# jameshensman/pyvb

Hardware: AMD Instinct MI355X
Metric: VB update iterations/sec (T=10k, D=64, N=1024 LDS); ELBO rel-err vs NumPy (higher is better)
Workload: dtype f64; 1 GPU; LDS T=10000 D=64 K=64, 1024 replicates per GPU (BASELINE configs[2]); replicates_total=1024, parallelism=replicates sharded over 1 GPU(s), collective=none (1 GPU), degraded=False

## Files before the change

### pyvb_amd/csrc/api.hip

```cpp
#include "common.h"
#include <cstdarg>
#include <cstdio>
#include <cstdlib>
#include <cstring>
#include <cmath>
#include <vector>
#include <mutex>
#include <dlfcn.h>

static thread_local char g_err[512] = "";

void pyvb_set_error(const char* fmt, ...) {
    va_list ap; va_start(ap, fmt);
    vsnprintf(g_err, sizeof(g_err), fmt, ap);
    va_end(ap);
}

int pyvb_hip_fail(hipError_t e, const char* what, const char* file, int line) {
    pyvb_set_error("HIP error %d (%s) in %s at %s:%d", (int)e, hipGetErrorString(e), what, file, line);
    return PYVB_E_HIP;
}

TimedLaunch::TimedLaunch(pyvb_lds* h_, int k_, hipStream_t s_) : h(h_), slot(-1), s(s_ ? s_ : h_->stream) {
    if (!h->timing) return;
// ... 610 lines not shown
        const double* Sm = S.data() + m * D * D;
        double s = 0.0;
        for (size_t j = 0; j < D && s == s; ++j) {
            for (size_t i = j; i < D; ++i) {
                double v = Sm[i * D + j];
                for (size_t k = 0; k < j; ++k) v -= L[i * D + k] * L[j * D + k];
                if (i == j) {
                    if (!(v > 0.0)) { s = NAN; break; }
                    L[j * D + j] = sqrt(v);
                    s += log(v);
                } else L[i * D + j] = v / L[j * D + j];
            }
        }
        lnd[m] = s;
    }
    HIPCHK(hipMemcpyAsync(h->lnd_x, lnd.data(), lnd.size() * sizeof(double), hipMemcpyHostToDevice, h->stream));
    HIPCHK(hipStreamSynchronize(h->stream));
    h->st.lnd_x_pending = false;
    return PYVB_OK;
}

static int ensure_gains(pyvb_lds* h) {
    if (h->st.gains_valid) return PYVB_OK;
    int rc;
    if (h->dense) {
        if ((rc = ensure_expect(h))) return rc;
        if ((rc = launch_dense_pre(h))) return rc;
    }
    if ((rc = launch_prep(h))) return rc;
    h->st.gains_formed();
    return PYVB_OK;
}

static void adopt_classes(pyvb_lds* h) {
    double* t = h->Sigma; h->Sigma = h->Sigma_new; h->Sigma_new = t;
    t = h->qld_x; h->qld_x = h->qld_x_new; h->qld_x_new = t;
    t = h->lnd_x; h->lnd_x = h->lnd_x_new; h->lnd_x_new = t;
    h->st.classes_adopted(h->n_active < h->N);
}

static int ensure_stats(pyvb_lds* h) {
    LdsState& st = h->st;
    if (st.stats_valid) return PYVB_OK;
    if (!st.classes_valid) {
        pyvb_set_error("the posterior covariances of the X_t are undefined before the first complete sweep "
                       "(run pyvb_lds_sweep, or give them with pyvb_lds_set_posterior_classes)");
        return PYVB_E_STALE;
    }
    if (st.mixed_cov || (st.gains_valid && st.fresh_count != 0 && st.fresh_count != h->T)) {
        pyvb_set_error("%d of %d X_t were updated since the parameters changed: their covariances differ; sweep all states first",
                       st.fresh_count, h->T);
        return PYVB_E_STALE;
    }
    int rc = launch_stats(h, !st.sxx_valid);
    if (rc) return rc;
    if ((rc = launch_moments(h, st.sxx_valid))) return rc;
    st.stats_valid = true;
    return PYVB_OK;
}

static int ensure_resid(pyvb_lds* h, int which) {
    bool& valid = which == 0 ? h->st.resQ_valid : h->st.resR_valid;
    if (valid) return PYVB_OK;
    int rc = ensure_stats(h);
    if (rc) return rc;
    if ((rc = h->dense ? launch_wresid(h, which, 0, h->st.sg_valid[which]) : launch_resid(h, which))) return rc;
    valid = true;
    return PYVB_OK;
}

static int sweep(pyvb_lds* h, int direction, bool keep_x) {
    int rc = ensure_gains(h);
    if (rc) return rc;
    const bool read_cache = direction == PYVB_BACKWARD && h->st.u_valid;
    if ((rc = launch_sweep(h, direction, h->st.cur, read_cache, keep_x))) return rc;
    h->st.sweep_ran(direction, read_cache, !h->big);
    if (h->st.all_fresh()) adopt_classes(h);
    return PYVB_OK;
}

int pyvb_lds_sweep(pyvb_lds* h, int direction) {
    ENTER(h);
    ARGCHK(direction == PYVB_FORWARD || direction == PYVB_BACKWARD, "direction must be PYVB_FORWARD or PYVB_BACKWARD");
    IDLE(h);
    return sweep(h, direction, true);
}

int pyvb_lds_update_x(pyvb_lds* h, int t) {
    ENTER(h);
    ARGCHK(t >= 0 && t < h->T, "t out of range");
    IDLE(h);
    int rc = ensure_gains(h);
    if (rc) return rc;
    if ((rc = launch_step(h, t))) return rc;
    h->st.x_changed();
    if (h->st.node_fresh(t)) adopt_classes(h);
    return PYVB_OK;
}

int pyvb_lds_update_columns(pyvb_lds* h, int which, int col_begin, int col_end) {
    ENTER(h);
    ARGCHK(which == 0 || which == 1, "which must be 0 (A) or 1 (C)");
    ARGCHK(col_begin >= 0 && col_begin < col_end && col_end <= h->D, "bad column range");
    IDLE(h);
    int rc = ensure_stats(h);
    if (rc) return rc;
    if (h->dense) {
        if ((rc = ensure_expect(h))) return rc;
        if ((rc = launch_cols_dense(h, which, col_begin, col_end))) return rc;
    } else if ((rc = launch_cols(h, which, col_begin, col_end))) return rc;
    h->st.columns_updated(which, h->dense && col_begin == 0 && col_end == h->D);
    return PYVB_OK;
}

int pyvb_lds_update_A(pyvb_lds* h) { ARGCHK(h, "handle is NULL"); return pyvb_lds_update_columns(h, 0, 0, h->D); }
int pyvb_lds_update_C(pyvb_lds* h) { ARGCHK(h, "handle is NULL"); return pyvb_lds_update_columns(h, 1, 0, h->D); }

static int update_noise(pyvb_lds* h, int which) {
    int rc;
    if (h->dense) {
        if ((rc = ensure_stats(h))) return rc;
        if ((rc = launch_wresid(h, which, 1, h->st.sg_valid[which]))) return rc;
    } else {
        if ((rc = ensure_resid(h, which))) return rc;
        if ((rc = launch_noise(h, which))) return rc;
    }
    h->st.noise_updated(which);
    return PYVB_OK;
}
// ... 310 lines not shown
```

### pyvb_amd/csrc/common.h

```cpp
#pragma once
#include <cstdint>
#include "host.h"

struct pyvb_comm;
typedef double d4 __attribute__((ext_vector_type(4)));
typedef double d2 __attribute__((ext_vector_type(2)));

struct Layout {
    int D, K, DT, KT, DP, KP, DS, KS;
    int QR;
    size_t oFn, oBn, oGp;
    size_t oS0, oS2, oqr, ow0;
    size_t gains_total;
    size_t stats_total;
    size_t oSxx, oSx1x, oSyx;
};

__host__ __device__ static inline int xpos(int d) { return (d & ~15) | ((d & 3) << 2) | ((d >> 2) & 3); }

__host__ __device__ static inline size_t pos_nat(int i, int j, int S) {
    return ((size_t)((i >> 4) * S + (j >> 2)) * 64) + (j & 3) * 16 + (i & 15);
}
__host__ __device__ static inline size_t pos_perm(int i, int j, int S) {
    int s = 2 * (j >> 3) + (j & 1), q = (j & 7) >> 1;
// ... 50 lines not shown
    double *A_mean, *A_var, *C_mean, *C_var;
    double *Q_a, *Q_b, *R_a, *R_b;
    double *qld_A, *qld_C;
    double *lnd_A, *lnd_C;
    int bound;
    Priors pri;
    double *pri_block;
    double *Sigma, *qld_x;
    double *Sigma_new, *qld_x_new;
    double *lnd_x, *lnd_x_new;
    double *gains;
    double *scratch;
    int *warm;
    double *zeros;
    double *trash;
    double *U;
    double *stats; int nchunk, chunk_len;
    int W;
    double *sxx;
    double *mom;
    double *resQ, *resR;
    double *elbo, *elbo_sum;
    int *status;
    unsigned char *active;
    unsigned char *active_host;
    int n_active;
    int *status_host, *reported;
    LdsState st;
    DeviceBuffers mem;
    bool timing; KernelTimer timers[PYVB_K_COUNT]; int timing_errors;
    pyvb_comm* comm; int rank, world;
    bool dense;
    double *Q_w, *R_w;
    double *Qbar, *Rbar;
    double *lnd;
    double *QA, *RC;
    double *trA, *trC;
    double *A_cov, *C_cov;
    double *SyyF;
    double *RQ, *RR;
    double *ldm;
    double *SG;
    bool has_missing;
    double *Yobs, *Yvar, *Yqld, *Yent;
    double *Ylnd, *YentX;
    double *Yld, *YcovS;
    hipStream_t side;
    hipEvent_t ev_params, ev_elbo;
    bool elbo_in_flight;
    double* elbo_hist; int hist_count;
};
#define PYVB_ELBO_HISTORY 4096

int launch_prep(pyvb_lds* h);
int launch_sweep(pyvb_lds* h, int direction, int src, bool read_cache, bool keep_x);
int launch_step(pyvb_lds* h, int t);
int launch_syy(pyvb_lds* h);
int launch_permute(pyvb_lds* h, const double* src, double* dst, int to_internal);
int launch_carry(pyvb_lds* h, const double* src, double* dst, size_t per);
int launch_stats(pyvb_lds* h, bool with_sxx);
int launch_moments(pyvb_lds* h, bool sxx_from_sweep);
int launch_observe(pyvb_lds* h);
int launch_cols(pyvb_lds* h, int which, int c0, int c1, int fuse = 0);
int launch_resid(pyvb_lds* h, int which);
int launch_noise(pyvb_lds* h, int which);
int launch_elbo(pyvb_lds* h, hipStream_t stream = nullptr);
int launch_elbo_sum(pyvb_lds* h, double* out = nullptr, hipStream_t stream = nullptr);
int launch_prep_big(pyvb_lds* h);
int big_prepare_kernels();
int launch_sweep_big(pyvb_lds* h, int direction, int src, bool cached);
int launch_step_big(pyvb_lds* h, int t);
int launch_stats_big(pyvb_lds* h);
int launch_cols_big(pyvb_lds* h, int which, int c0, int c1, int fuse);
int launch_wexpect(pyvb_lds* h);
int launch_dense_pre(pyvb_lds* h);
int launch_cols_dense(pyvb_lds* h, int which, int c0, int c1);
int launch_wresid(pyvb_lds* h, int which, int update, bool use_sg);
int launch_syy_full(pyvb_lds* h);
int launch_elbo_dense(pyvb_lds* h, hipStream_t stream = nullptr);
int launch_colvar_to_cov(pyvb_lds* h);
int launch_cov_to_colvar(pyvb_lds* h);
int launch_cov_observe(pyvb_lds* h);
int launch_cov_convert(pyvb_lds* h, int which, double* dense, int n0, int count, int to_packed);
int launch_wexpect_big(pyvb_lds* h);
int launch_dense_pre_big(pyvb_lds* h);
int launch_cols_dense_big(pyvb_lds* h, int which, int c0, int c1);
int launch_wresid_big(pyvb_lds* h, int which, int update, bool use_sg);
int launch_syy_full_big(pyvb_lds* h);
int launch_missing_init(pyvb_lds* h, const double* Yq0, const double* Yrowvar0);
int launch_impute(pyvb_lds* h);
int launch_syy_missing(pyvb_lds* h);
int launch_impute_dense(pyvb_lds* h);
int launch_missing_ent_dense(pyvb_lds* h, int diag_cov);

struct pyvb_comm {
    void* nccl;
    pyvb_host_allreduce_fn fn; void* user;
    double* host; size_t cap;
};
int pyvb_comm_create(pyvb_comm** comm, const char id[128], int rank, int world);
int pyvb_comm_create_host(pyvb_comm** comm, pyvb_host_allreduce_fn fn, void* user);
void pyvb_comm_free(pyvb_comm* comm);
int pyvb_allreduce_f64(pyvb_comm* comm, double* buf, size_t count, hipStream_t stream);

#define PYVB_EVENT_POOL 2048
struct EventPair { hipEvent_t e0, e1; int kernel; };
struct TimedLaunch {
    pyvb_lds* h; int slot; hipStream_t s;
    TimedLaunch(pyvb_lds* h_, int k_, hipStream_t s_ = nullptr);
    ~TimedLaunch();
};
void pyvb_timing_resolve(pyvb_lds* h);
```

### pyvb_amd/csrc/host.h

```cpp
#pragma once
#include <hip/hip_runtime.h>
#include <cstddef>
#include <cstring>
#include <vector>
#include "../../include/pyvb_hip.h"

void pyvb_set_error(const char* fmt, ...);
int pyvb_hip_fail(hipError_t e, const char* what, const char* file, int line);
#define HIPCHK(x) do { hipError_t _e = (x); if (_e != hipSuccess) return pyvb_hip_fail(_e, #x, __FILE__, __LINE__); } while (0)
#define ARGCHK(cond, msg) do { if (!(cond)) { pyvb_set_error("%s", msg); return PYVB_E_ARG; } } while (0)
#define ENTER_DEVICE(h) do { ARGCHK(h, "handle is NULL"); HIPCHK(hipSetDevice((h)->device)); } while (0)
#define CREATE_TRY(x, DESTROY, h) do { rc = (x); if (rc != PYVB_OK) { DESTROY(h); return rc; } } while (0)
#define CREATE_TRYHIP(x, DESTROY, h) do { hipError_t _e = (x); if (_e != hipSuccess) { rc = pyvb_hip_fail(_e, #x, __FILE__, __LINE__); DESTROY(h); return rc; } } while (0)

struct DeviceBuffers {
    std::vector<void*> owned;
    int alloc(void** p, size_t bytes, int fill_byte = 0) {
        HIPCHK(hipMalloc(p, bytes));
        owned.push_back(*p);
        HIPCHK(hipMemset(*p, fill_byte, bytes));
        return PYVB_OK;
    }
    int zeros(double** p, size_t n) { return alloc((void**)p, n * sizeof(double)); }
    void release(void* p) {
        for (size_t i = 0; i < owned.size(); ++i)
            if (owned[i] == p) { (void)hipFree(p); owned[i] = owned.back(); owned.pop_back(); return; }
    }
    void release_all() { for (void* p : owned) (void)hipFree(p); owned.clear(); }
};

static inline int to_device(hipStream_t s, double* dst, const double* src, size_t n) {
    if (!src) return PYVB_OK;
    HIPCHK(hipMemcpyAsync(dst, src, n * sizeof(double), hipMemcpyHostToDevice, s));
    return PYVB_OK;
}
static inline int to_host(hipStream_t s, double* dst, const double* src, size_t n) {
    if (!dst) return PYVB_OK;
    HIPCHK(hipMemcpyAsync(dst, src, n * sizeof(double), hipMemcpyDeviceToHost, s));
    return PYVB_OK;
}

struct LdsState {
    int T;
    int cur;
    bool gains_valid;
    bool expect_valid;
    bool stats_valid;
    bool resQ_valid, resR_valid;
    bool sg_valid[2];
    bool u_valid;
    bool sxx_valid;
    unsigned char* fresh;
    int fresh_count;
    bool mixed_cov;
    bool classes_valid;
    bool lnd_x_pending;
    int x_park;
    bool cls_parked_other;

    void params_touched() {
        if (gains_valid && fresh_count != 0 && fresh_count != T) mixed_cov = true;
        gains_valid = false;
        u_valid = false;
    }
    void sums_stale() { stats_valid = false; resQ_valid = resR_valid = false; sg_valid[0] = sg_valid[1] = false; }

    void parameters_changed() { params_touched(); resQ_valid = resR_valid = false; }
    void columns_changed() { parameters_changed(); sg_valid[0] = sg_valid[1] = false; }
    void noise_changed() { expect_valid = false; params_touched(); }
    void noise_updated(int which) {
        if (which != 1) resQ_valid = true;
        if (which != 0) resR_valid = true;
        noise_changed();
    }
    void columns_updated(int which, bool sums_all) {
        if (which != 1) { sg_valid[0] = sums_all; resQ_valid = false; }
        if (which != 0) { sg_valid[1] = sums_all; resR_valid = false; }
        params_touched();
    }
    void outputs_changed() { u_valid = false; sums_stale(); }
    void x_changed() { u_valid = false; sxx_valid = false; sums_stale(); }
    void classes_set() { lnd_x_pending = true; classes_valid = true; sums_stale(); }
    void gains_formed() { gains_valid = true; memset(fresh, 0, T); fresh_count = 0; }
    bool node_fresh(int t) {
        if (fresh[t]) return false;
        fresh[t] = 1;
        if (++fresh_count < T) return false;
        mixed_cov = false;
        return true;
    }
    bool all_fresh() {
        const bool adopt = fresh_count < T;
        if (adopt) { memset(fresh, 1, T); fresh_count = T; }
        mixed_cov = false;
        return adopt;
    }
    void sweep_ran(int direction, bool read_cache, bool fused_sxx) {
        cur = 1 - cur;
        sxx_valid = read_cache && fused_sxx;
        u_valid = direction == PYVB_FORWARD;
        sums_stale();
    }
    void classes_adopted(bool some_parked) {
        lnd_x_pending = false;
        classes_valid = true;
        if (some_parked) cls_parked_other = !cls_parked_other;
    }
    void parked_here() { x_park = cur; cls_parked_other = false; }
};

struct PcaState {
    bool full_valid, lin_valid;
    bool res_valid;
    bool z_pending;
    bool z0_done;
    bool xlazy; long vlo, vhi;
    int part_chunks;

    void inputs_changed() { full_valid = lin_valid = false; res_valid = false; }
    void z_requested() { z_pending = true; z0_done = false; }
    void z_written() { z_pending = false; z0_done = false; }
    void linear_step() { full_valid = false; res_valid = false; }
};
```

### pyvb_amd/csrc/k_params.hip

```cpp
#include "params.h"

__global__ void __launch_bounds__(256) k_moments(ParamArgs a) {
    const int n = blockIdx.x, tid = threadIdx.x, D = a.D, K = a.K, T = a.T, DP = a.L.DP;
    if (!a.active[n]) return;
    const double* P = a.part + (size_t)n * a.nchunk * a.L.stats_total;
    const double* S = a.Sigma + (size_t)n * 3 * D * D;
    const double* x0 = a.X + (size_t)n * T * DP;
    const double* xL = x0 + (size_t)(T - 1) * DP;
    double* mo = a.mom + (size_t)n * mom_total(D, K);
    const double nint = (double)(T - 2);
    for (int idx = tid; idx < D * D; idx += 256) {
        const int i = idx / D, j = idx % D;
        double xx = 0.0, h = 0.0;
        for (int ch = 0; ch < a.nchunk; ++ch) {
            const double* Pc = P + (size_t)ch * a.L.stats_total;
            if (!a.sxx) xx += Pc[a.L.oSxx + (size_t)i * DP + j];
            h += Pc[a.L.oSx1x + (size_t)i * DP + j];
        }
        if (a.sxx) {
            xx = x0[xpos(i)] * x0[xpos(j)] + xL[xpos(i)] * xL[xpos(j)];
#pragma unroll 8
            for (int w = 0; w < a.W; ++w) xx += a.sxx[((size_t)n * a.W + w) * DP * DP + (size_t)i * DP + j];
        }
        const double s0 = S[idx], s1 = S[D * D + idx], s2 = S[2 * D * D + idx];
        mo[MOM_GA(D, K) + idx] = xx - xL[xpos(i)] * xL[xpos(j)] + s0 + nint * s1;
        mo[MOM_GC(D, K) + idx] = xx + s0 + nint * s1 + s2;
        mo[MOM_HA(D, K) + idx] = h;
        if (i == j) mo[MOM_DP(D, K) + i] = xx - x0[xpos(i)] * x0[xpos(i)] + nint * s1 + s2;
    }
    for (int idx = tid; idx < K * D; idx += 256) {
        const int k = idx / D, j = idx % D;
        double h = 0.0;
        for (int ch = 0; ch < a.nchunk; ++ch) h += P[(size_t)ch * a.L.stats_total + a.L.oSyx + (size_t)k * DP + j];
        mo[MOM_HC(D, K) + idx] = h;
    }
}

template <int NW>
__device__ __forceinline__ double blk_sum(double v, double* red) {
    v = wave_sum(v);
    if constexpr (NW == 1) return v;
    else {
        __syncthreads();
        if ((threadIdx.x & 63) == 0) red[threadIdx.x >> 6] = v;
        __syncthreads();
        return red[0] + red[1];
    }
}

template <int NW>
__global__ void __launch_bounds__(64 * NW) k_noise(ParamArgs a) {
    __shared__ double red[2];
    const int WHICH = a.which0 + blockIdx.y;
    const int n = blockIdx.x, lane = threadIdx.x;
    if (!a.active[n]) return;
    const int dim = WHICH == 0 ? a.D : a.K;
    const double* res = (WHICH == 0 ? a.resQ : a.resR) + (size_t)n * dim;
    const double* b0 = WHICH == 0 ? a.pri.Q_b0 : a.pri.R_b0;
    double* qb = (WHICH == 0 ? a.Q_b : a.R_b) + (size_t)n * dim;
    const bool live = lane < dim;
    double r = live ? res[lane] : 0.0;
    if (a.noise == PYVB_NOISE_GAMMA) {
        r = blk_sum<NW>(r, red);
        if (live) qb[lane] = b0[0] + r;
    } else if (live) {
        qb[lane] = b0[lane] + r;
    }
}

__device__ __forceinline__ double gamma_llb(double a0, double b0, double qa, double qb) {
    const double Elnx = digamma_pos(qa) - log(qb);
    double ret = (a0 - 1.0) * Elnx - lgamma(a0) + a0 * log(b0) - b0 * (qa / qb);
    ret -= (qa - 1.0) * Elnx - lgamma(qa) + qa * log(qb) - qb * (qa / qb);
    return ret;
}

template <int NW>
__global__ void __launch_bounds__(64 * NW) k_elbo(ParamArgs a) {
    __shared__ double red[2];
    const int n = blockIdx.x, lane = threadIdx.x, D = a.D, K = a.K, T = a.T;
    if (!a.active[n]) return;
    const double* S0 = a.Sigma + (size_t)n * 3 * D * D;
    const double* x0 = a.X + (size_t)n * T * a.L.DP;
    const bool exact = a.bound == PYVB_BOUND_EXACT;
    const double* qx = (exact ? a.lnd_x : a.qld_x) + (size_t)n * 3;
    double qbar = 0.0, rbar = 0.0, lnq = 0.0, lnr = 0.0, rq = 0.0, rr = 0.0, lq = 0.0, lr = 0.0;
// ... 70 lines not shown
        };
        la = column(D, a.pri.A_pp, a.pri.A_pm, a.A_mean + (size_t)n * D * D, a.A_var + (size_t)n * D * D, a.pri.A_obs,
                    (exact ? a.lnd_A : a.qld_A)[(size_t)n * D + i], a.pri.A_pld[i]);
        lc = column(K, a.pri.C_pp, a.pri.C_pm, a.C_mean + (size_t)n * K * D, a.C_var + (size_t)n * D * K, a.pri.C_obs,
                    (exact ? a.lnd_C : a.qld_C)[(size_t)n * D + i], a.pri.C_pld[i]);
    }
    const double LA = blk_sum<NW>(la, red), LC = blk_sum<NW>(lc, red);
    if (lane == 0) {
        double* o = a.elbo + (size_t)n * 6;
        o[0] = LX; o[1] = LY; o[2] = LA; o[3] = LC; o[4] = LQ; o[5] = LR;
    }
}

struct SumArgs { const double* elbo; double* out; const unsigned char* active; int N; };
__global__ void __launch_bounds__(256) k_elbo_sum(SumArgs a) {
    __shared__ double red[256 * 6];
    const int tid = threadIdx.x;
    double s[6] = {0, 0, 0, 0, 0, 0};
    for (int n = tid; n < a.N; n += 256)
        if (a.active[n])
            for (int p = 0; p < 6; ++p) s[p] += a.elbo[(size_t)n * 6 + p];
    for (int p = 0; p < 6; ++p) red[p * 256 + tid] = s[p];
    __syncthreads();
    if (tid < 6) {
        double t = 0.0;
        for (int i = 0; i < 256; ++i) t += red[tid * 256 + i];
        a.out[tid] = t;
    }
}

template <int NW>
__global__ void __launch_bounds__(64 * NW) k_observe(ParamArgs a) {
    __shared__ double red[2];
    const int WHICH = blockIdx.y, n = blockIdx.x, lane = threadIdx.x, D = a.D;
    if (!a.active[n]) return;
    const int rows = WHICH == 0 ? a.D : a.K;
    double* M = (WHICH == 0 ? a.A_mean : a.C_mean) + (size_t)n * rows * D;
    double* V = (WHICH == 0 ? a.A_var : a.C_var) + (size_t)n * D * rows;
    const double* obs = WHICH == 0 ? a.pri.A_obs : a.pri.C_obs;
    for (int i = 0; i < D; ++i) {
        const double ob = lane < rows ? obs[(size_t)lane * D + i] : 0.0;
        const int nknown = (int)blk_sum<NW>((lane < rows && ob == ob) ? 1.0 : 0.0, red);
        if (nknown == rows && lane < rows) { M[(size_t)lane * D + i] = ob; V[(size_t)i * rows + lane] = 0.0; }
    }
}

ParamArgs make_args(pyvb_lds* h) {
    ParamArgs a;
    a.part = h->stats; a.nchunk = h->nchunk; a.mom = h->mom; a.Sigma = h->Sigma; a.qld_x = h->qld_x; a.X = h->X[h->st.cur]; a.Syy = h->Syy;
    a.A_mean = h->A_mean; a.A_var = h->A_var; a.C_mean = h->C_mean; a.C_var = h->C_var;
    a.Q_a = h->Q_a; a.Q_b = h->Q_b; a.R_a = h->R_a; a.R_b = h->R_b; a.qld_A = h->qld_A; a.qld_C = h->qld_C;
    a.resQ = h->resQ; a.resR = h->resR; a.elbo = h->elbo; a.pri = h->pri; a.Yent = h->has_missing ? h->Yent : nullptr;
    a.lnd_A = h->lnd_A; a.lnd_C = h->lnd_C; a.lnd_x = h->lnd_x; a.YentX = h->has_missing ? h->YentX : nullptr; a.bound = h->bound;
    a.N = h->N; a.T = h->T; a.D = h->D; a.K = h->K; a.noise = h->noise; a.L = h->L; a.c0 = 0; a.c1 = h->D; a.which0 = 0; a.fuse = 0; a.sxx = nullptr; a.W = 1;
    a.active = h->active;
    return a;
}

int launch_observe(pyvb_lds* h) {
    ParamArgs a = make_args(h);
    if (h->big) hipLaunchKernelGGL(k_observe<2>, dim3(h->N, 2), dim3(128), 0, h->stream, a);
    else hipLaunchKernelGGL(k_observe<1>, dim3(h->N, 2), dim3(64), 0, h->stream, a);
    HIPCHK(hipGetLastError());
    return PYVB_OK;
}

int launch_moments(pyvb_lds* h, bool sxx_from_sweep) {
    ParamArgs a = make_args(h);
    a.sxx = sxx_from_sweep ? h->sxx : nullptr;
    a.W = h->W;
    TimedLaunch tl(h, PYVB_K_PARAMS);
    hipLaunchKernelGGL(k_moments, dim3(h->N), dim3(256), 0, h->stream, a);
    HIPCHK(hipGetLastError());
    return PYVB_OK;
}

int launch_noise(pyvb_lds* h, int which) {
    ParamArgs a = make_args(h);
    a.which0 = which == 1 ? 1 : 0;
    TimedLaunch tl(h, PYVB_K_PARAMS);
    if (h->big) hipLaunchKernelGGL(k_noise<2>, dim3(h->N, which == 2 ? 2 : 1), dim3(128), 0, h->stream, a);
    else hipLaunchKernelGGL(k_noise<1>, dim3(h->N, which == 2 ? 2 : 1), dim3(64), 0, h->stream, a);
    HIPCHK(hipGetLastError());
    return PYVB_OK;
}

int launch_elbo(pyvb_lds* h, hipStream_t stream) {
    ParamArgs a = make_args(h);
    if (!stream) stream = h->stream;
    TimedLaunch tl(h, PYVB_K_ELBO, stream);
    if (h->big) hipLaunchKernelGGL(k_elbo<2>, dim3(h->N), dim3(128), 0, stream, a);
    else hipLaunchKernelGGL(k_elbo<1>, dim3(h->N), dim3(64), 0, stream, a);
    HIPCHK(hipGetLastError());
    return PYVB_OK;
}

int launch_elbo_sum(pyvb_lds* h, double* out, hipStream_t stream) {
    SumArgs a; a.elbo = h->elbo; a.out = out ? out : h->elbo_sum; a.active = h->active; a.N = h->N;
    hipLaunchKernelGGL(k_elbo_sum, dim3(1), dim3(256), 0, stream ? stream : h->stream, a);
    HIPCHK(hipGetLastError());
    return PYVB_OK;
}
```

### pyvb_amd/csrc/k_sweep.hip

```cpp
#include "common.h"

struct SweepArgs {
    const double* Xold; double* Xnew; const double* Y; const double* gains; const int* warm;
    const double *A_mean, *C_mean;
    const double *QA, *RC;
    double* trash;
    double* U;
    double* Sxx;
    int N, T, D, K, dir;
    int W;
    const unsigned char* active;
    int keep_x;
    Layout L;
};

#define MFMA(a, b, c) __builtin_amdgcn_mfma_f64_16x16x4f64((a), (b), (c), 0, 0, 0)

template <class NB>
__device__ __forceinline__ double boundary_update(bool first, const double* g, const Layout& L, const double* Am, const double* Cm,
                                                  int D, int K, int lane, NB nb, const double* y, double* vs,
                                                  const double* QA = nullptr, const double* RC = nullptr) {
    const double* qb = g + L.oqr;
    const double* rb = qb + 64;
    double v = 0.0;
    if (QA) {
        if (lane < D) {
            if (first) {
                v = g[L.ow0 + lane];
                for (int i = 0; i < D; ++i) v += QA[(size_t)i * D + lane] * nb(i);
            } else {
                for (int j = 0; j < D; ++j) v += QA[(size_t)lane * D + j] * nb(j);
            }
            for (int k = 0; k < K; ++k) v += RC[(size_t)k * D + lane] * y[k];
        }
    } else if (lane < D) {
        if (first) {
            v = g[L.ow0 + lane];
            for (int i = 0; i < D; ++i) v += Am[(size_t)i * D + lane] * (qb[i] * nb(i));
        } else {
            double s = 0.0;
            for (int j = 0; j < D; ++j) s += Am[(size_t)lane * D + j] * nb(j);
            v = qb[lane] * s;
        }
        for (int k = 0; k < K; ++k) v += Cm[(size_t)k * D + lane] * (rb[k] * y[k]);
    }
    vs[lane] = v;
    __syncthreads();
    const double* S = g + (first ? L.oS0 : L.oS2);
    double s = 0.0;
    if (lane < D)
        for (int j = 0; j < D; ++j) s += S[(size_t)j * L.DP + lane] * vs[j];
    __syncthreads();
    return s;
}

template <int DT, int KT, bool FULL, int MODE, bool SPLIT>
__global__ void __launch_bounds__(64) k_sweep(SweepArgs a) {
    constexpr int DS = 4 * DT, KS = 4 * KT, DP = 16 * DT;
    __shared__ double gl[MODE == 2 ? DP * 17 : DT * KS * 64];
    __shared__ double xs[64];
    __shared__ double vs[64];
    const int n = blockIdx.x, w = SPLIT ? blockIdx.y : 0, lane = threadIdx.x, c = lane & 15, q = lane >> 4;
    if (!a.active[n]) return;
    const int T = a.T, D = a.D, K = a.K;
    const bool fwd = (a.dir == 0);
// ... 184 lines not shown
        if constexpr (MODE == 1) store_x(trash + 64);
        load_o(jstart, mo);
        for (int j = jstart; j < Lseg; ++j) {
            d4 acc[DT];
            {
#pragma unroll
                for (int m = 0; m < DT; ++m) acc[m] = d4{0.0, 0.0, 0.0, 0.0};
                int goff = lane;
                asm volatile("" : "+v"(goff));
#pragma unroll
                for (int s = 0; s < KS; ++s)
#pragma unroll
                    for (int m = 0; m < DT; ++m) acc[m] = MFMA(gl[(m * KS + s) * 64 + goff], yv[s >> 1][s & 1], acc[m]);
                __builtin_amdgcn_sched_barrier(0);
                load_y(j + 1, yv);
                store_x(out_pending);
                __builtin_amdgcn_sched_barrier(0);
            }
            mul_resident(acc, rn, x);
            {
                if constexpr (MODE == 1) {
                    __builtin_amdgcn_sched_barrier(0);
                    double* ur = u_row(j);
#pragma unroll
                    for (int m = 0; m < DT; ++m) *reinterpret_cast<d4*>(ur + (m * 4 + q) * 4) = acc[m];
                    __builtin_amdgcn_sched_barrier(0);
                }
                mul_resident(acc, ip, mo);
                __builtin_amdgcn_sched_barrier(0);
                load_o(j + 1, mo);
                __builtin_amdgcn_sched_barrier(0);
            }
            finish_step(j, acc);
        }
        store_x(out_pending);
        }
        const int clast = (Tw - 1) / Lseg;
        __builtin_amdgcn_s_barrier();
        if (c == clast) {
#pragma unroll
            for (int m = 0; m < DT; ++m)
#pragma unroll
                for (int r = 0; r < 4; ++r) xs[16 * m + 4 * r + q] = x[m][r];
        }
        __builtin_amdgcn_fence(__ATOMIC_RELEASE, "workgroup");
        __builtin_amdgcn_s_barrier();
        __builtin_amdgcn_fence(__ATOMIC_ACQUIRE, "workgroup");
    }

    if (!SPLIT || w == ((Tint > 0) ? (Tint - 1) / Lw : 0)) {
        const double s = boundary_update(!fwd, g, L, Am, Cm, D, K, lane, [&](int j) { return xs[j]; },
                                         Yn + (size_t)t_last * K, vs, QAm, RCm);
        if (lane < DP) Xn[(size_t)t_last * DP + xpos(lane)] = (lane < D) ? s : 0.0;
    }
}

struct StepArgs {
    double* X; const double* Y; const double* gains; const double *A_mean, *C_mean, *QA, *RC;
    const unsigned char* active;
    int N, T, D, K, t;
    Layout L;
};

__global__ void __launch_bounds__(64) k_step(StepArgs a) {
    const int n = blockIdx.x, lane = threadIdx.x;
    if (!a.active[n]) return;
    const int T = a.T, D = a.D, K = a.K, t = a.t, DP = a.L.DP;
    const Layout& L = a.L;
    const double* g = a.gains + (size_t)n * L.gains_total;
    double* X = a.X + (size_t)n * T * DP;
    const double* y = a.Y + ((size_t)n * T + t) * K;
    const int cls = (t == 0) ? 0 : (t == T - 1 ? 2 : 1);
    const int row = lane % DP;
    if (cls != 1) {
        __shared__ double vs[64];
        const double* nbr = X + (size_t)(cls == 0 ? 1 : T - 2) * DP;
        const double s = boundary_update(cls == 0, g, L, a.A_mean + (size_t)n * D * D, a.C_mean + (size_t)n * K * D, D, K, lane,
                                         [&](int j) { return nbr[xpos(j)]; }, y, vs,
                                         a.QA ? a.QA + (size_t)n * D * D : nullptr, a.RC ? a.RC + (size_t)n * K * D : nullptr);
        if (lane < DP) X[(size_t)t * DP + xpos(lane)] = (lane < D) ? s : 0.0;
        return;
    }
    const int DS = L.DS, KS = L.KS;
    double s = 0.0;
    for (int j = 0; j < D; ++j) s += g[L.oFn + pos_nat(row, j, DS)] * X[(size_t)(t - 1) * DP + xpos(j)];
    for (int j = 0; j < D; ++j) s += g[L.oBn + pos_nat(row, j, DS)] * X[(size_t)(t + 1) * DP + xpos(j)];
    for (int k = 0; k < K; ++k) s += g[L.oGp + pos_perm(row, k, KS)] * y[k];
    if (lane < DP) X[(size_t)t * DP + xpos(lane)] = (lane < D) ? s : 0.0;
}

template <int DT, int KT>
static int launch_sweep_t(pyvb_lds* h, const SweepArgs& a, bool read_cache) {
    const bool full = h->D == 16 * DT && h->K == 16 * KT;
    const int mode = a.dir == PYVB_FORWARD ? 1 : (read_cache ? 2 : 0);
#define PYVB_SWEEP_CASE(F, M) do { if (h->W > 1) hipLaunchKernelGGL((k_sweep<DT, KT, F, M, true>), dim3(h->N, h->W), dim3(64), 0, h->stream, a); \
                                   else hipLaunchKernelGGL((k_sweep<DT, KT, F, M, false>), dim3(h->N), dim3(64), 0, h->stream, a); } while (0)
    if (full) { if (mode == 1) PYVB_SWEEP_CASE(true, 1); else if (mode == 2) PYVB_SWEEP_CASE(true, 2); else PYVB_SWEEP_CASE(true, 0); }
    else { if (mode == 1) PYVB_SWEEP_CASE(false, 1); else if (mode == 2) PYVB_SWEEP_CASE(false, 2); else PYVB_SWEEP_CASE(false, 0); }
#undef PYVB_SWEEP_CASE
    return PYVB_OK;
}

int launch_sweep(pyvb_lds* h, int direction, int src, bool read_cache, bool keep_x) {
    if (h->big) return launch_sweep_big(h, direction, src, read_cache);
    SweepArgs a;
    a.keep_x = (keep_x || direction != PYVB_FORWARD) ? 1 : 0;
    a.W = h->W;
    a.Xold = h->X[src]; a.Xnew = h->X[1 - src]; a.Y = h->Y; a.gains = h->gains; a.warm = h->warm;
    a.trash = h->trash; a.U = h->U; a.Sxx = h->sxx; a.A_mean = h->A_mean; a.C_mean = h->C_mean;
    a.QA = h->dense ? h->QA : nullptr; a.RC = h->dense ? h->RC : nullptr;
    a.N = h->N; a.T = h->T; a.D = h->D; a.K = h->K; a.dir = direction; a.L = h->L; a.active = h->active;
    {
        TimedLaunch tl(h, direction == PYVB_FORWARD ? PYVB_K_SWEEP_FWD : PYVB_K_SWEEP_BWD);
        switch (h->L.DT * 10 + h->L.KT) {
            case 11: launch_sweep_t<1, 1>(h, a, read_cache); break;
            case 12: launch_sweep_t<1, 2>(h, a, read_cache); break;
            case 14: launch_sweep_t<1, 4>(h, a, read_cache); break;
            case 21: launch_sweep_t<2, 1>(h, a, read_cache); break;
            case 22: launch_sweep_t<2, 2>(h, a, read_cache); break;
            case 24: launch_sweep_t<2, 4>(h, a, read_cache); break;
            case 41: launch_sweep_t<4, 1>(h, a, read_cache); break;
            case 42: launch_sweep_t<4, 2>(h, a, read_cache); break;
            case 44: launch_sweep_t<4, 4>(h, a, read_cache); break;
            default: pyvb_set_error("unsupported tile shape"); return PYVB_E_ARG;
        }
    }
    HIPCHK(hipGetLastError());
    return PYVB_OK;
}

struct PermArgs { const double* src; double* dst; size_t rows; int D, DP, to_internal; };
__global__ void __launch_bounds__(256) k_permute(PermArgs a) {
    const int per = a.DP > 64 ? 128 : 64;
    const size_t row = (size_t)blockIdx.x * (256 / per) + (threadIdx.x / per);
    const int d = threadIdx.x % per;
    if (row >= a.rows || d >= a.DP) return;
    if (a.to_internal) a.dst[row * a.DP + xpos(d)] = (d < a.D) ? a.src[row * a.D + d] : 0.0;
    else if (d < a.D) a.dst[row * a.D + d] = a.src[row * a.DP + xpos(d)];
}

int launch_permute(pyvb_lds* h, const double* src, double* dst, int to_internal) {
    PermArgs a; a.src = src; a.dst = dst; a.rows = (size_t)h->N * h->T; a.D = h->D; a.DP = h->L.DP; a.to_internal = to_internal;
    const size_t per_block = a.DP > 64 ? 2 : 4;
    hipLaunchKernelGGL(k_permute, dim3((unsigned)((a.rows + per_block - 1) / per_block)), dim3(256), 0, h->stream, a);
    HIPCHK(hipGetLastError());
    return PYVB_OK;
}

struct CarryArgs { const double* src; double* dst; const unsigned char* active; size_t per; };
__global__ void __launch_bounds__(256) k_carry(CarryArgs a) {
    const int n = blockIdx.y;
    if (a.active[n]) return;
    const double* s = a.src + (size_t)n * a.per;
    double* d = a.dst + (size_t)n * a.per;
    for (size_t i = (size_t)blockIdx.x * 256 + threadIdx.x; i < a.per; i += (size_t)gridDim.x * 256) d[i] = s[i];
}

int launch_carry(pyvb_lds* h, const double* src, double* dst, size_t per) {
    CarryArgs a; a.src = src; a.dst = dst; a.active = h->active; a.per = per;
    const size_t blocks = (per + 255) / 256;
    hipLaunchKernelGGL(k_carry, dim3((unsigned)(blocks < 64 ? blocks : 64), h->N), dim3(256), 0, h->stream, a);
    HIPCHK(hipGetLastError());
    return PYVB_OK;
}

int launch_step(pyvb_lds* h, int t) {
// ... 11 lines not shown
```

### pyvb_amd/csrc/params.h

```cpp
#pragma once
#include "common.h"

#define LN2PI 1.8378770664093453

struct ParamArgs {
    const double* part; int nchunk; const double* Sigma; const double* qld_x; const double* X; const double* Syy;
    double* mom;
    const double* sxx;
    int W;
    double *A_mean, *A_var, *C_mean, *C_var, *Q_a, *Q_b, *R_a, *R_b, *qld_A, *qld_C;
    double *lnd_A, *lnd_C;
    const double* lnd_x;
    double *resQ, *resR, *elbo;
    const double* Yent;
    const double* YentX;
    int bound;
    Priors pri;
    int N, T, D, K, noise;
    int c0, c1;
    int fuse;
    const unsigned char* active;
    int which0;
    Layout L;
};

__host__ __device__ static inline size_t mom_total(int D, int K) { return (size_t)3 * D * D + (size_t)K * D + D; }
#define MOM_GA(D, K) ((size_t)0)
#define MOM_GC(D, K) ((size_t)(D) * (D))
#define MOM_HA(D, K) ((size_t)2 * (D) * (D))
#define MOM_HC(D, K) ((size_t)3 * (D) * (D))
#define MOM_DP(D, K) ((size_t)3 * (D) * (D) + (size_t)(K) * (D))

__device__ __forceinline__ double wave_sum(double v) {
#pragma unroll
    for (int o = 32; o > 0; o >>= 1) v += __shfl_xor(v, o, 64);
    return v;
}

__device__ __forceinline__ double bcast(double v, int j) {
    const int lo = __builtin_amdgcn_readlane(__double2loint(v), j);
    const int hi = __builtin_amdgcn_readlane(__double2hiint(v), j);
    return __hiloint2double(hi, lo);
}

__device__ static inline double digamma_pos(double x) {
    if (!(x - x == 0.0) || x < -4.5e15) return x > 0 ? x : __builtin_nan("");
    double r = 0.0;
    if (x < -64.0) { r = -M_PI / tan(M_PI * x); x = 1.0 - x; }
    while (x < 10.0) { r -= 1.0 / x; x += 1.0; }
    const double f = 1.0 / (x * x);
    const double ser = f * (1.0 / 12 - f * (1.0 / 120 - f * (1.0 / 252 - f * (1.0 / 240 - f * (1.0 / 132 - f * (691.0 / 32760 - f / 12))))));
    return r + log(x) - 0.5 / x - ser;
}


ParamArgs make_args(pyvb_lds* h);
```

Before: 87.74 VB iterations/s per 1024 replicates (whole job).

## Fuse sufficient-statistics accumulation into the backward sweep kernel for D=64

Adds a k_sweep_stats kernel that, during the cached backward sweep, stages freshly computed X_t and Y_t tiles in LDS and accumulates the cross-moment (Sx1x, Syx) and Sxx statistics with MFMA as it goes. Segment-boundary cross terms and the endpoint terms are then added in k_moments, and the separate launch_stats pass is skipped when the fused path ran. This targets the extra full pass over X and Y in memory that the stats kernel needed. In exchange it adds per-step LDS barriers and extra MFMA work inside the latency-bound recurrence, plus new state tracking (fused_valid).

```diff
diff --git a/pyvb_amd/csrc/api.hip b/pyvb_amd/csrc/api.hip
--- a/pyvb_amd/csrc/api.hip
+++ b/pyvb_amd/csrc/api.hip
@@ -686,9 +686,9 @@
                        st.fresh_count, h->T);
         return PYVB_E_STALE;
     }
-    int rc = launch_stats(h, !st.sxx_valid);
-    if (rc) return rc;
-    if ((rc = launch_moments(h, st.sxx_valid))) return rc;
+    int rc;
+    if (!st.fused_valid && (rc = launch_stats(h, !st.sxx_valid))) return rc;
+    if ((rc = launch_moments(h, st.sxx_valid, st.fused_valid))) return rc;
     st.stats_valid = true;
     return PYVB_OK;
 }
@@ -708,7 +708,7 @@
     if (rc) return rc;
     const bool read_cache = direction == PYVB_BACKWARD && h->st.u_valid;
     if ((rc = launch_sweep(h, direction, h->st.cur, read_cache, keep_x))) return rc;
-    h->st.sweep_ran(direction, read_cache, !h->big);
+    h->st.sweep_ran(direction, read_cache, !h->big, fused_stats_sweep(h));
     if (h->st.all_fresh()) adopt_classes(h);
     return PYVB_OK;
 }
diff --git a/pyvb_amd/csrc/common.h b/pyvb_amd/csrc/common.h
--- a/pyvb_amd/csrc/common.h
+++ b/pyvb_amd/csrc/common.h
@@ -126,6 +126,18 @@
 };
 #define PYVB_ELBO_HISTORY 4096
 
+__host__ __device__ static inline int fused_part_len(int T) { return ((((T - 2) + 1) / 2) + 15) & ~15; }
+__host__ __device__ static inline int fused_segment_start(int T, int w, int c) {
+    const int Tint = T - 2, Lw = fused_part_len(T), ow = w * Lw;
+    const int Tw = (Tint - ow < Lw) ? Tint - ow : Lw;
+    const int Lseg = (Tw + 15) >> 4;
+    return (Tw > 0 && c * Lseg < Tw) ? ow + c * Lseg : -1;
+}
+#define PYVB_FUSED_MIN_INTERIOR 32
+static inline bool fused_stats_sweep(const pyvb_lds* h) {
+    return !h->big && h->L.DT == 4 && h->W == 1 && h->T - 2 >= PYVB_FUSED_MIN_INTERIOR;
+}
+
 int launch_prep(pyvb_lds* h);
 int launch_sweep(pyvb_lds* h, int direction, int src, bool read_cache, bool keep_x);
 int launch_step(pyvb_lds* h, int t);
@@ -133,7 +145,7 @@
 int launch_permute(pyvb_lds* h, const double* src, double* dst, int to_internal);
 int launch_carry(pyvb_lds* h, const double* src, double* dst, size_t per);
 int launch_stats(pyvb_lds* h, bool with_sxx);
-int launch_moments(pyvb_lds* h, bool sxx_from_sweep);
+int launch_moments(pyvb_lds* h, bool sxx_from_sweep, bool all_from_sweep);
 int launch_observe(pyvb_lds* h);
 int launch_cols(pyvb_lds* h, int which, int c0, int c1, int fuse = 0);
 int launch_resid(pyvb_lds* h, int which);
diff --git a/pyvb_amd/csrc/host.h b/pyvb_amd/csrc/host.h
--- a/pyvb_amd/csrc/host.h
+++ b/pyvb_amd/csrc/host.h
@@ -50,6 +50,7 @@
     bool sg_valid[2];
     bool u_valid;
     bool sxx_valid;
+    bool fused_valid;
     unsigned char* fresh;
     int fresh_count;
     bool mixed_cov;
@@ -78,8 +79,8 @@
         if (which != 0) { sg_valid[1] = sums_all; resR_valid = false; }
         params_touched();
     }
-    void outputs_changed() { u_valid = false; sums_stale(); }
-    void x_changed() { u_valid = false; sxx_valid = false; sums_stale(); }
+    void outputs_changed() { u_valid = false; fused_valid = false; sums_stale(); }
+    void x_changed() { u_valid = false; sxx_valid = fused_valid = false; sums_stale(); }
     void classes_set() { lnd_x_pending = true; classes_valid = true; sums_stale(); }
     void gains_formed() { gains_valid = true; memset(fresh, 0, T); fresh_count = 0; }
     bool node_fresh(int t) {
@@ -95,9 +96,10 @@
         mixed_cov = false;
         return adopt;
     }
-    void sweep_ran(int direction, bool read_cache, bool fused_sxx) {
+    void sweep_ran(int direction, bool read_cache, bool fused_sxx, bool fused_all) {
         cur = 1 - cur;
         sxx_valid = read_cache && fused_sxx;
+        fused_valid = sxx_valid && fused_all;
         u_valid = direction == PYVB_FORWARD;
         sums_stale();
     }
diff --git a/pyvb_amd/csrc/k_params.hip b/pyvb_amd/csrc/k_params.hip
--- a/pyvb_amd/csrc/k_params.hip
+++ b/pyvb_amd/csrc/k_params.hip
@@ -1,8 +1,19 @@
 #include "params.h"
 
 __global__ void __launch_bounds__(256) k_moments(ParamArgs a) {
+    __shared__ double bx[33][2][64];
     const int n = blockIdx.x, tid = threadIdx.x, D = a.D, K = a.K, T = a.T, DP = a.L.DP;
     if (!a.active[n]) return;
+    const int nsum = a.fused ? 1 : a.nchunk;
+    if (a.fused) {
+        const double* Xr = a.X + (size_t)n * T * DP;
+        for (int idx = tid; idx < 33 * 2 * 64; idx += 256) {
+            const int pr = idx >> 7, lo = (idx >> 6) & 1, d = idx & 63;
+            const int st = pr < 32 ? fused_segment_start(T, pr >> 4, pr & 15) : T - 2;
+            bx[pr][lo][d] = (st >= 0 && d < D) ? Xr[(size_t)(T - 2 - st + 1 - lo) * DP + xpos(d)] : 0.0;
+        }
+        __syncthreads();
+    }
     const double* P = a.part + (size_t)n * a.nchunk * a.L.stats_total;
     const double* S = a.Sigma + (size_t)n * 3 * D * D;
     const double* x0 = a.X + (size_t)n * T * DP;
@@ -12,10 +23,14 @@
     for (int idx = tid; idx < D * D; idx += 256) {
         const int i = idx / D, j = idx % D;
         double xx = 0.0, h = 0.0;
-        for (int ch = 0; ch < a.nchunk; ++ch) {
+        for (int ch = 0; ch < nsum; ++ch) {
             const double* Pc = P + (size_t)ch * a.L.stats_total;
             if (!a.sxx) xx += Pc[a.L.oSxx + (size_t)i * DP + j];
             h += Pc[a.L.oSx1x + (size_t)i * DP + j];
+        }
+        if (a.fused) {
+#pragma unroll 3
+            for (int pr = 0; pr < 33; ++pr) h += bx[pr][0][i] * bx[pr][1][j];
         }
         if (a.sxx) {
             xx = x0[xpos(i)] * x0[xpos(j)] + xL[xpos(i)] * xL[xpos(j)];
@@ -31,7 +46,11 @@
     for (int idx = tid; idx < K * D; idx += 256) {
         const int k = idx / D, j = idx % D;
         double h = 0.0;
-        for (int ch = 0; ch < a.nchunk; ++ch) h += P[(size_t)ch * a.L.stats_total + a.L.oSyx + (size_t)k * DP + j];
+        for (int ch = 0; ch < nsum; ++ch) h += P[(size_t)ch * a.L.stats_total + a.L.oSyx + (size_t)k * DP + j];
+        if (a.fused) {
+            const double* Yn = a.Y + (size_t)n * T * K;
+            h += Yn[k] * x0[xpos(j)] + Yn[(size_t)(T - 1) * K + k] * xL[xpos(j)];
+        }
         mo[MOM_HC(D, K) + idx] = h;
     }
 }
@@ -208,7 +227,7 @@
     a.Q_a = h->Q_a; a.Q_b = h->Q_b; a.R_a = h->R_a; a.R_b = h->R_b; a.qld_A = h->qld_A; a.qld_C = h->qld_C;
     a.resQ = h->resQ; a.resR = h->resR; a.elbo = h->elbo; a.pri = h->pri; a.Yent = h->has_missing ? h->Yent : nullptr;
     a.lnd_A = h->lnd_A; a.lnd_C = h->lnd_C; a.lnd_x = h->lnd_x; a.YentX = h->has_missing ? h->YentX : nullptr; a.bound = h->bound;
-    a.N = h->N; a.T = h->T; a.D = h->D; a.K = h->K; a.noise = h->noise; a.L = h->L; a.c0 = 0; a.c1 = h->D; a.which0 = 0; a.fuse = 0; a.sxx = nullptr; a.W = 1;
+    a.N = h->N; a.T = h->T; a.D = h->D; a.K = h->K; a.noise = h->noise; a.L = h->L; a.c0 = 0; a.c1 = h->D; a.which0 = 0; a.fuse = 0; a.sxx = nullptr; a.W = 1; a.fused = 0; a.Y = h->Y;
     a.active = h->active;
     return a;
 }
@@ -221,10 +240,11 @@
     return PYVB_OK;
 }
 
-int launch_moments(pyvb_lds* h, bool sxx_from_sweep) {
+int launch_moments(pyvb_lds* h, bool sxx_from_sweep, bool all_from_sweep) {
     ParamArgs a = make_args(h);
     a.sxx = sxx_from_sweep ? h->sxx : nullptr;
     a.W = h->W;
+    a.fused = (sxx_from_sweep && all_from_sweep) ? 1 : 0;
     TimedLaunch tl(h, PYVB_K_PARAMS);
     hipLaunchKernelGGL(k_moments, dim3(h->N), dim3(256), 0, h->stream, a);
     HIPCHK(hipGetLastError());
diff --git a/pyvb_amd/csrc/k_sweep.hip b/pyvb_amd/csrc/k_sweep.hip
--- a/pyvb_amd/csrc/k_sweep.hip
+++ b/pyvb_amd/csrc/k_sweep.hip
@@ -11,6 +11,8 @@
     int W;
     const unsigned char* active;
     int keep_x;
+    double* part;
+    size_t part_stride;
     Layout L;
 };
 
@@ -301,6 +303,217 @@
         const double s = boundary_update(!fwd, g, L, Am, Cm, D, K, lane, [&](int j) { return xs[j]; },
                                          Yn + (size_t)t_last * K, vs, QAm, RCm);
         if (lane < DP) Xn[(size_t)t_last * DP + xpos(lane)] = (lane < D) ? s : 0.0;
+    }
+}
+
+template <int KT, bool FULL>
+__global__ void __launch_bounds__(128) k_sweep_stats(SweepArgs a) {
+    constexpr int DT = 4, DS = 16, DP = 64, TS = DP * 17, HB = 3 * TS;
+    __shared__ double tl[2 * HB];
+    __shared__ double xs[2][64];
+    __shared__ double vs[2][64];
+    const int n = blockIdx.x, w = threadIdx.x >> 6, lane = threadIdx.x & 63, c = lane & 15, q = lane >> 4;
+    if (!a.active[n]) return;
+    const int T = a.T, D = a.D, K = a.K;
+    const Layout& L = a.L;
+    const double* g = a.gains + (size_t)n * L.gains_total;
+    const double* Xo = a.Xold + (size_t)n * T * DP;
+    double* Xn = a.Xnew + (size_t)n * T * DP;
+    const double* Yn = a.Y + (size_t)n * T * K;
+
+    double rn[DT][DS];
+    {
+        const double* Rn = g + L.oBn;
+#pragma unroll
+        for (int m = 0; m < DT; ++m)
+#pragma unroll
+            for (int s = 0; s < DS; ++s) rn[m][s] = Rn[(m * DS + s) * 64 + lane];
+    }
+    for (int i = threadIdx.x; i < 2 * HB; i += 128) tl[i] = 0.0;
+
+    const int Tint = T - 2, Lw = fused_part_len(T), ow = w * Lw;
+    const int Tw = (Tint - ow < Lw) ? Tint - ow : Lw;
+    const int J = a.warm[n * 2 + 1];
+
+    const double* Am = a.A_mean + (size_t)n * D * D;
+    const double* Cm = a.C_mean + (size_t)n * K * D;
+    const double* QAm = a.QA ? a.QA + (size_t)n * D * D : nullptr;
+    const double* RCm = a.RC ? a.RC + (size_t)n * K * D : nullptr;
+    {
+        const double* xo = Xo + (size_t)(T - 2) * DP;
+        const double s = boundary_update(false, g, L, Am, Cm, D, K, lane, [&](int j) { return xo[xpos(j)]; },
+                                         Yn + (size_t)(T - 1) * K, vs[w], QAm, RCm);
+        if (w == 0) Xn[(size_t)(T - 1) * DP + xpos(lane)] = (lane < D) ? s : 0.0;
+        xs[w][lane] = (lane < D) ? s : 0.0;
+    }
+    __syncthreads();
+
+    const int Lseg = (Tw + 15) >> 4;
+    const int Lseg0 = Lw >> 4, Lseg1 = (Tint - Lw + 15) >> 4;
+    const int reach0 = 15 * Lseg0, reach1 = Lw + 15 * Lseg1;
+    const int js0 = -(J < reach0 ? J : reach0), js1 = -(J < reach1 ? J : reach1);
+    const int jstart = js0 < js1 ? js0 : js1;
+    const int jend = Lseg0;
+    const int cL = c * Lseg;
+    const int before = ow + cL;
+    const int jc = -(J < before ? J : before);
+    d4 x[DT];
+#pragma unroll
+    for (int m = 0; m < DT; ++m)
+#pragma unroll
+        for (int r = 0; r < 4; ++r) x[m][r] = (jc == -before) ? xs[w][16 * m + 4 * r + q] : 0.0;
+    const int tbase = T - 2 - before, tsafe = T - 2;
+    auto active = [&](int j) { int tt = cL + j; return j >= jc && j < Lseg && tt < Tw; };
+    double* const trash = a.trash + (size_t)n * 256 + 128 * w;
+    double* out_pending = trash;
+    const double* const Un = a.U + (size_t)n * T * DP;
+    auto load_u = [&](int j, d4* dst) {
+        const double* p = Un + (size_t)(active(j) ? tbase - j : tsafe) * DP;
+#pragma unroll
+        for (int m = 0; m < DT; ++m) dst[m] = *reinterpret_cast<const d4*>(p + (m * 4 + q) * 4);
+    };
+    auto load_y = [&](int j, d4* dst) {
+        const double* p = Yn + (size_t)(active(j) ? tbase - j : tsafe) * K;
+        int klast = K - 1;
+        if constexpr (!FULL) asm volatile("" : "+v"(klast));
+#pragma unroll
+        for (int m = 0; m < KT; ++m) {
+            const int d0 = (m * 4 + q) * 4;
+            if constexpr (FULL) dst[m] = *reinterpret_cast<const d4*>(p + d0);
+            else {
+#pragma unroll
+                for (int r = 0; r < 4; ++r) dst[m][r] = p[d0 + r < klast ? d0 + r : klast];
+            }
+        }
+    };
+    auto store_x = [&](double* out) {
+#pragma unroll
+        for (int m = 0; m < DT; ++m) *reinterpret_cast<d4*>(out + (m * 4 + q) * 4) = x[m];
+    };
+
+    const int lb = c * 17 + q;
+    int xa[4];
+    xa[0] = lb + (w ? 2 : 0) * 272; xa[1] = lb + (w ? 3 : 1) * 272; xa[2] = lb + (w ? 1 : 2) * 272; xa[3] = lb + (w ? 0 : 3) * 272;
+    int aa[2];
+    aa[0] = lb + (w ? 2 * TS : TS); aa[1] = lb + (w ? 2 * TS : 0);
+    d4 st[DT][4], sx[5];
+#pragma unroll
+    for (int m = 0; m < DT; ++m)
+#pragma unroll
+        for (int i = 0; i < 4; ++i) st[m][i] = d4{0.0, 0.0, 0.0, 0.0};
+#pragma unroll
+    for (int i = 0; i < 5; ++i) sx[i] = d4{0.0, 0.0, 0.0, 0.0};
+
+    auto operands = [&](int g8, int p, double* xo, double* ao) {
+        const int off = (g8 >> 2) * HB + 4 * (g8 & 3);
+#pragma unroll
+        for (int i = 0; i < 4; ++i) xo[i] = tl[xa[i] + off + p * TS];
+#pragma unroll
+        for (int m = 0; m < DT; ++m) ao[m] = tl[aa[p] + off + m * 272];
+    };
+    auto accumulate = [&](int p) {
+        double xo[2][4], ao[2][4];
+        operands(0, p, xo[0], ao[0]);
+#pragma unroll
+        for (int g8 = 0; g8 < 8; ++g8) {
+            if (g8 < 7) operands(g8 + 1, p, xo[(g8 + 1) & 1], ao[(g8 + 1) & 1]);
+            __builtin_amdgcn_sched_barrier(0);
+            const double* xv = xo[g8 & 1];
+            const double* av = ao[g8 & 1];
+#pragma unroll
+            for (int m = 0; m < DT; ++m)
+#pragma unroll
+                for (int i = 0; i < 4; ++i) st[m][i] = MFMA(av[m], xv[i], st[m][i]);
+            sx[0] = MFMA(xv[0], xv[0], sx[0]);
+            sx[1] = MFMA(xv[1], xv[1], sx[1]);
+            sx[2] = MFMA(xv[0], xv[1], sx[2]);
+            sx[3] = MFMA(xv[0], xv[2], sx[3]);
+            sx[4] = MFMA(xv[1], xv[3], sx[4]);
+            __builtin_amdgcn_sched_barrier(0);
+        }
+    };
+    auto lds_barrier = [&]() {
+        __builtin_amdgcn_fence(__ATOMIC_RELEASE, "workgroup", "local");
+        __builtin_amdgcn_s_barrier();
+        __builtin_amdgcn_fence(__ATOMIC_ACQUIRE, "workgroup", "local");
+    };
+
+    d4 ub[DT];
+    double* const mine = tl + w * HB;
+    load_u(jstart, ub);
+    store_x(trash);
+    for (int j = jstart; j < jend; j += 2) {
+#pragma unroll
+        for (int p = 0; p < 2; ++p) {
+            d4 acc[DT], yv[KT];
+#pragma unroll
+            for (int m = 0; m < DT; ++m) acc[m] = ub[m];
+            __builtin_amdgcn_sched_barrier(0);
+            load_y(j + p, yv);
+            load_u(j + p + 1, ub);
+            store_x(out_pending);
+            __builtin_amdgcn_sched_barrier(0);
+#pragma unroll
+            for (int s = 0; s < DS; ++s)
+#pragma unroll
+                for (int m = 0; m < DT; ++m) acc[m] = MFMA(rn[m][s], x[s >> 2][s & 3], acc[m]);
+            const bool act = active(j + p);
+            const bool keep = act && j + p >= 0;
+#pragma unroll
+            for (int m = 0; m < DT; ++m)
+#pragma unroll
+                for (int r = 0; r < 4; ++r) x[m][r] = act ? acc[m][r] : x[m][r];
+            out_pending = (keep && (a.keep_x || before + j + p == Tint - 1)) ? Xn + (size_t)(tbase - (j + p)) * DP : trash;
+            lds_barrier();
+#pragma unroll
+            for (int m = 0; m < DT; ++m)
+#pragma unroll
+                for (int r = 0; r < 4; ++r) mine[p * TS + (16 * m + 4 * r + q) * 17 + c] = keep ? x[m][r] : 0.0;
+#pragma unroll
+            for (int m = 0; m < KT; ++m)
+#pragma unroll
+                for (int r = 0; r < 4; ++r) mine[2 * TS + (16 * m + 4 * q + r) * 17 + c] = yv[m][r];
+            lds_barrier();
+            accumulate(p);
+        }
+    }
+    store_x(out_pending);
+
+    {
+        double* P = a.part + (size_t)n * a.part_stride + (w ? L.oSyx : L.oSx1x);
+        const int mlim = w ? KT : DT;
+        const int pm[4] = {w ? 2 : 0, w ? 3 : 1, w ? 1 : 2, w ? 0 : 3};
+#pragma unroll
+        for (int m = 0; m < DT; ++m)
+            if (m < mlim) {
+#pragma unroll
+                for (int i = 0; i < 4; ++i)
+#pragma unroll
+                    for (int e = 0; e < 4; ++e) P[(size_t)(16 * m + 4 * e + q) * DP + 16 * pm[i] + c] = st[m][i][e];
+            }
+        double* Sn = a.Sxx + (size_t)n * DP * DP;
+        const int ta[5] = {0, 1, 0, 0, 1}, tb[5] = {0, 1, 1, 2, 3};
+#pragma unroll
+        for (int i = 0; i < 5; ++i)
+#pragma unroll
+            for (int e = 0; e < 4; ++e) {
+                const int row = 16 * pm[ta[i]] + 4 * e + q, col = 16 * pm[tb[i]] + c;
+                Sn[(size_t)row * DP + col] = sx[i][e];
+                if (ta[i] != tb[i]) Sn[(size_t)col * DP + row] = sx[i][e];
+            }
+    }
+
+    const int clast = (Tw - 1) / Lseg;
+    if (c == clast) {
+#pragma unroll
+        for (int m = 0; m < DT; ++m)
+#pragma unroll
+            for (int r = 0; r < 4; ++r) xs[w][16 * m + 4 * r + q] = x[m][r];
+    }
+    __syncthreads();
+    {
+        const double s = boundary_update(true, g, L, Am, Cm, D, K, lane, [&](int j) { return xs[w][j]; }, Yn, vs[w], QAm, RCm);
+        if (w == 1) Xn[xpos(lane)] = (lane < D) ? s : 0.0;
     }
 }
 
@@ -350,6 +563,20 @@
     return PYVB_OK;
 }
 
+static int launch_sweep_stats(pyvb_lds* h, const SweepArgs& a) {
+    const bool full = h->D == 64 && h->K == 16 * h->L.KT;
+#define PYVB_FUSED_CASE(KT) do { if (full) hipLaunchKernelGGL((k_sweep_stats<KT, true>), dim3(h->N), dim3(128), 0, h->stream, a); \
+                                 else hipLaunchKernelGGL((k_sweep_stats<KT, false>), dim3(h->N), dim3(128), 0, h->stream, a); } while (0)
+    switch (h->L.KT) {
+        case 1: PYVB_FUSED_CASE(1); break;
+        case 2: PYVB_FUSED_CASE(2); break;
+        case 4: PYVB_FUSED_CASE(4); break;
+        default: pyvb_set_error("unsupported tile shape"); return PYVB_E_ARG;
+    }
+#undef PYVB_FUSED_CASE
+    return PYVB_OK;
+}
+
 int launch_sweep(pyvb_lds* h, int direction, int src, bool read_cache, bool keep_x) {
     if (h->big) return launch_sweep_big(h, direction, src, read_cache);
     SweepArgs a;
@@ -359,8 +586,13 @@
     a.trash = h->trash; a.U = h->U; a.Sxx = h->sxx; a.A_mean = h->A_mean; a.C_mean = h->C_mean;
     a.QA = h->dense ? h->QA : nullptr; a.RC = h->dense ? h->RC : nullptr;
     a.N = h->N; a.T = h->T; a.D = h->D; a.K = h->K; a.dir = direction; a.L = h->L; a.active = h->active;
+    a.part = h->stats; a.part_stride = (size_t)h->nchunk * h->L.stats_total;
     {
         TimedLaunch tl(h, direction == PYVB_FORWARD ? PYVB_K_SWEEP_FWD : PYVB_K_SWEEP_BWD);
+        if (direction == PYVB_BACKWARD && read_cache && fused_stats_sweep(h)) {
+            int rc = launch_sweep_stats(h, a);
+            if (rc) return rc;
+        } else
         switch (h->L.DT * 10 + h->L.KT) {
             case 11: launch_sweep_t<1, 1>(h, a, read_cache); break;
             case 12: launch_sweep_t<1, 2>(h, a, read_cache); break;
diff --git a/pyvb_amd/csrc/params.h b/pyvb_amd/csrc/params.h
--- a/pyvb_amd/csrc/params.h
+++ b/pyvb_amd/csrc/params.h
@@ -8,6 +8,8 @@
     double* mom;
     const double* sxx;
     int W;
+    int fused;
+    const double* Y;
     double *A_mean, *A_var, *C_mean, *C_var, *Q_a, *Q_b, *R_a, *R_b, *qld_A, *qld_C;
     double *lnd_A, *lnd_C;
     const double* lnd_x;
```

Result: slower. 83.29 VB iterations/s per 1024 replicates (whole job) (-5.1%).
